# underdoc-wang/ST-MGCN

Hardware: NVIDIA H100
Metric: region-timesteps/sec (fwd+bwd) (higher is better)
Workload: dtype f32

## Files before the change

### st-mgcn_b200/csrc/lstm16.cu

```cuda
#include "tc16.cuh"
#include <cuda.h>
#include <stdlib.h>
#include <string.h>

using namespace stmgcn;
using namespace stmgcn::tc;

namespace {

constexpr int kTileM = 128;
constexpr int kHid = 64;
constexpr int kGateCols = 256;
constexpr int kMaxC = 4;
constexpr int kWTileBytes = kGateCols * 128;
constexpr int kATileBytes = kTile16Bytes;

__host__ __device__ __forceinline__ uint32_t blocked_off(uint32_t tile, uint32_t row, uint32_t unit) {
    return tile * 8192u + (unit >> 2) * 512u + row * 4u + (unit & 3u);
}
__host__ __device__ __forceinline__ int64_t blocked_slice(int n_tiles) { return (int64_t)n_tiles * kTileM * kHid; }

__device__ __forceinline__ float gate_scale(int col) { return (col & 3) == 2 ? kNeg2Log2e : kNegLog2e; }
__device__ __forceinline__ float exp_arg_(float a) { return ex2_ftz_(fminf(a, 43.28f)); }
__device__ __forceinline__ void lstm_cell_fwd8(float ai, float af, float ag, float ao, float cp, float& c, float& h) {
// ... 230 lines not shown
                    wg_wait<0>();
                }
                wg_fence_regs(acc);
            } else {
#pragma unroll
                for (int k = 0; k < 128; ++k) acc[k] = 0.f;
            }
            if (issuer) bulk_wait_group_read0();
            bar_sync(kFBarWg + wg, 128);
            if (!L0) {
                if (issuer) mbar_arrive(&tail->empty[wg]);
                ++n_below;
            }
            float* c_row = p.cs + (int64_t)t * cslice + cbase + blocked_off(0, 0, q >> 1);
            const bool store_h = valid && t == p.t_len - 1 && p.h_f32 != nullptr;
            float* h_row = p.h_f32 + (store_h ? r * (uint32_t)kHid + (uint32_t)(q >> 1) : 0u);
#pragma unroll
            for (int j0 = 0; j0 < 32; j0 += kFCellBatch) {
                float4 v[kFCellBatch], bv[kFCellBatch];
                float cp[kFCellBatch], cn[kFCellBatch], hn[kFCellBatch];
#pragma unroll
                for (int k = 0; k < kFCellBatch; ++k) v[k] = frag_to_gates(acc, j0 + k, odd);
#pragma unroll
                for (int k = 0; k < kFCellBatch; ++k) {
                    const int col = 4 * (2 * (j0 + k) + (q >> 1));
                    bv[k] = *reinterpret_cast<const float4*>(&tail->bias[col]);
                    cp[k] = c_sm[128 * (j0 + k)];
                }
#pragma unroll
                for (int k = 0; k < kFCellBatch; ++k) {
                    const int col = 4 * (2 * (j0 + k) + (q >> 1));
                    const float4 a = gate_args<CIN>(v[k], bv[k], xs, wih_s, col, kC);
                    lstm_cell_fwd8(a.x, a.y, a.z, a.w, cp[k], cn[k], hn[k]);
                }
#pragma unroll
                for (int k = 0; k < kFCellBatch; ++k) {
                    const int unit = 2 * (j0 + k) + (q >> 1);
                    c_sm[128 * (j0 + k)] = cn[k];
                    if (valid) c_row[blocked_off(0, 0, 2 * (j0 + k))] = cn[k];
                    if (store_h) h_row[2 * (j0 + k)] = hn[k];
                    const uint32_t off = sw128<2>(row_in_wg, (uint32_t)unit);
                    const __nv_bfloat16 hb = __float2bfloat16_rn(hn[k]);
                    *reinterpret_cast<__nv_bfloat16*>(h_sm + off) = hb;
                    if (PLANES == 2) *reinterpret_cast<__nv_bfloat16*>(h_sm + kHTileBytes + off) = __float2bfloat16_rn(hn[k] - __bfloat162float(hb));
                }
            }
            fence_proxy_async_smem();
            bar_sync(kFBarWg + wg, 128);
            if (issuer) {
                for (int pl = 0; pl < PLANES; ++pl)
                    tma_store_3d(&p.hp_map, h_sm + (size_t)pl * kHTileBytes, 0, row0, (p.layer * p.t_len + t) * PLANES + pl);
                bulk_commit_group();
            }
        }
    }
    if (issuer) bulk_wait_group_read0();
}

__global__ void lstm16_pack_kernel(const float* __restrict__ w_ih, const float* __restrict__ w_hh,
                                   const float* __restrict__ b_ih, const float* __restrict__ b_hh, int layer, int c_in,
                                   uint8_t* __restrict__ wimg, float* __restrict__ bias, float* __restrict__ wih_t) {
    const int nseg = layer == 0 ? 1 : 2;
    const int total = nseg * kGateCols * kHid;
    for (int e = blockIdx.x * blockDim.x + threadIdx.x; e < total; e += gridDim.x * blockDim.x) {
        const int s = e / (kGateCols * kHid), n = (e / kHid) % kGateCols, k = e % kHid;
        const int nat = (n & 3) * kHid + (n >> 2);
        const float* src = (layer > 0 && s == 0) ? w_ih : w_hh;
        const float v = src[(int64_t)nat * kHid + k];
        const __nv_bfloat16 h = __float2bfloat16_rn(v);
        const __nv_bfloat16 l = __float2bfloat16_rn(v - __bfloat162float(h));
        const uint32_t off = sw128<2>((uint32_t)n, (uint32_t)k);
        *reinterpret_cast<__nv_bfloat16*>(wimg + (size_t)(s * 2) * kWTileBytes + off) = h;
        *reinterpret_cast<__nv_bfloat16*>(wimg + (size_t)(s * 2 + 1) * kWTileBytes + off) = l;
    }
    for (int n = blockIdx.x * blockDim.x + threadIdx.x; n < kGateCols; n += gridDim.x * blockDim.x) {
        const int nat = (n & 3) * kHid + (n >> 2);
        bias[n] = b_ih[nat] + b_hh[nat];
        if (layer == 0 && wih_t != nullptr)
            for (int c = 0; c < c_in; ++c) wih_t[c * kGateCols + n] = w_ih[(int64_t)nat * c_in + c];
    }
}


constexpr int kBWarpgroups = 2;
constexpr int kBThreads = kBWarpgroups * 128 + 128;
constexpr int kBCons = kBWarpgroups * 128;
constexpr uint32_t kBBarCons = 1;
constexpr uint32_t kBBarWg = 2;
constexpr int kBDbWarps = 2;
constexpr uint32_t kBBarDa = 4;
constexpr uint32_t kBDaThreads = kBCons + 32 * kBDbWarps;
constexpr uint32_t kBConsRegs = 240, kBProdRegs = 24;
constexpr int kBATiles = 4;

struct B16Tail {
    float bias[kGateCols];
    uint64_t a_full, a_empty, w_full;
};
constexpr size_t kBSmem = 1024 + 4 * (size_t)kWTileBytes + kBATiles * (size_t)kATileBytes + 2 * (size_t)kATileBytes + sizeof(B16Tail);
static_assert(kBSmem <= 232448, "lstm16 backward kernel exceeds the 227 KB shared-memory limit");

constexpr int kBMaxSteps = 64;
struct Bwd16Step {
    int32_t slice[2];
    int8_t src[2];
    int8_t first;
    int8_t store_dh;
    int32_t t;
    const float* c_prev;
    const float* dh_in;
    float* dx_out;
};
struct Bwd16Params {
    alignas(64) CUtensorMap maps[2];
    const uint8_t* zero_tile;
    const uint8_t* wimg;
    const float* bias;
    const float* wih;
    const float* xo;
    const float* sg;
    float* d_s;
    float* d_xo;
    int c_in, t_len, n_steps;
    int64_t b_inner;
    float* dh_rec;
    float* dc;
    float* dbp;
    float* dw_slice;
    int64_t rows;
    int n_tiles;
    Bwd16Step steps[kBMaxSteps];
};
static_assert(sizeof(Bwd16Params) <= 4096, "kernel parameter block exceeds 4 KB");

template <int PLANES, int NSEG>
__device__ __forceinline__ void bwd_recompute_mma(float (&g)[32], uint32_t a_u, uint32_t a_rows, uint32_t w_u, int c) {
#pragma unroll
    for (int s = 0; s < NSEG; ++s) {
        const uint64_t a_hi = desc16_k(a_u + (uint32_t)(s * 2) * kATileBytes + a_rows);
        const uint64_t a_lo = desc16_k(a_u + (uint32_t)(s * 2 + 1) * kATileBytes + a_rows);
        const uint64_t b_hi = desc16_k(w_u + (uint32_t)(s * 2) * kWTileBytes + (uint32_t)c * 8192u);
        const uint64_t b_lo = desc16_k(w_u + (uint32_t)(s * 2 + 1) * kWTileBytes + (uint32_t)c * 8192u);
#pragma unroll
        for (int kk = 0; kk < 4; ++kk) {
            wgmma_bf16_n64_t00(g, a_hi + 2 * kk, b_hi + 2 * kk, (s > 0 || kk > 0) ? 1u : 0u);
            if (PLANES == 2) {
                wgmma_bf16_n64_t00(g, a_hi + 2 * kk, b_lo + 2 * kk, 1u);
                wgmma_bf16_n64_t00(g, a_lo + 2 * kk, b_hi + 2 * kk, 1u);
            }
        }
    }
}

constexpr uint32_t kStepMN = 2048;

template <int PLANES, bool L0>
__device__ __forceinline__ void bwd_wgrad_mma(float (&wgr)[32], uint32_t wa_hi, uint32_t da_u) {
    const uint32_t wa_lo = wa_hi + kATileBytes;
#pragma unroll
    for (int ks = 0; ks < 8; ++ks) {
        const uint64_t ah = desc16_mn(wa_hi + ks * kStepMN, kATileBytes);
        const uint64_t al = desc16_mn(wa_lo + ks * kStepMN, kATileBytes);
        const uint64_t bh = desc16_mn(da_u + ks * kStepMN, kATileBytes);
        const uint64_t bl = desc16_mn(da_u + kATileBytes + ks * kStepMN, kATileBytes);
        wgmma_bf16_n64_t11(wgr, ah, bh, ks > 0 ? 1u : 0u);
        wgmma_bf16_n64_t11(wgr, ah, bl, 1u);
        if (PLANES == 2 || L0) wgmma_bf16_n64_t11(wgr, al, bh, 1u);
    }
}

template <int PLANES, int NSEG>
__device__ __forceinline__ void bwd_dgrad_mma(float (&dacc)[32 * NSEG], uint32_t da_u, uint32_t a_rows, uint32_t w_u, int c) {
    const uint64_t ah = desc16_k(da_u + a_rows), al = desc16_k(da_u + kATileBytes + a_rows);
#pragma unroll
    for (int kk = 0; kk < 4; ++kk) {
        const uint32_t wb = w_u + (uint32_t)c * 8192u + (uint32_t)kk * kStepMN;
        const uint64_t bh = desc16_mn(wb, 2 * kWTileBytes), bl = desc16_mn(wb + kWTileBytes, 2 * kWTileBytes);
        if constexpr (NSEG == 2) {
            wgmma_bf16_n128_t01(dacc, ah + 2 * kk, bh, 1u);
            if (PLANES == 2) wgmma_bf16_n128_t01(dacc, ah + 2 * kk, bl, 1u);
            wgmma_bf16_n128_t01(dacc, al + 2 * kk, bh, 1u);
        } else {
            wgmma_bf16_n64_t01(dacc, ah + 2 * kk, bh, 1u);
            if (PLANES == 2) wgmma_bf16_n64_t01(dacc, ah + 2 * kk, bl, 1u);
            wgmma_bf16_n64_t01(dacc, al + 2 * kk, bh, 1u);
        }
    }
}

__device__ __forceinline__ void bwd_wgrad_red(float* slice, const float (&wgr)[32], uint32_t rw0, int q, int c) {
#pragma unroll
    for (int j = 0; j < 8; ++j) {
        const uint32_t n = (uint32_t)(64 * c + 8 * j + 2 * q);
        red_add_f32x2(slice + (size_t)rw0 * kGateCols + n, wgr[4 * j], wgr[4 * j + 1]);
        red_add_f32x2(slice + (size_t)(rw0 + 8) * kGateCols + n, wgr[4 * j + 2], wgr[4 * j + 3]);
    }
}

template <int PLANES, int CIN>
__global__ void __launch_bounds__(kBThreads, 1) lstm16_bwd_kernel(const __grid_constant__ Bwd16Params p) {
    constexpr bool L0 = CIN > 0;
    constexpr int kC = (CIN == 1) ? 1 : kMaxC;
    constexpr int kNseg = L0 ? 1 : 2;
    extern __shared__ uint8_t smem_raw[];
    uint8_t* smem = smem_raw + smem_pad1024(smem_raw);
    uint8_t* w_sm = smem;
    uint8_t* a_sm = w_sm + 4 * (size_t)kWTileBytes;
    uint8_t* da_sm = a_sm + kBATiles * (size_t)kATileBytes;
    B16Tail* tail = (B16Tail*)(da_sm + 2 * (size_t)kATileBytes);
    float* wih_s = reinterpret_cast<float*>(w_sm + 2 * (size_t)kWTileBytes);
    const int tid = threadIdx.x;
    const int warp = tid >> 5;
    const int lane = tid & 31;
    constexpr int kProdWarp = kBWarpgroups * 4;

    if (tid == 0) {
        mbar_init(&tail->a_full, 1);
        mbar_init(&tail->a_empty, kBWarpgroups);
        mbar_init(&tail->w_full, 1);
        fence_barrier_init();
    }
    for (int i = tid; i < kGateCols; i += kBThreads) tail->bias[i] = p.bias[i] * gate_scale(i);
    if (L0) {
        for (int i = tid; i < p.c_in * kGateCols; i += kBThreads) wih_s[i] = p.wih[i] * gate_scale(i);
        for (int i = tid; i < 2 * kATileBytes / 16; i += kBThreads)
            reinterpret_cast<uint4*>(a_sm + 2 * (size_t)kATileBytes)[i] = make_uint4(0u, 0u, 0u, 0u);
        if (PLANES == 1)
            for (int i = tid; i < kATileBytes / 16; i += kBThreads)
                reinterpret_cast<uint4*>(a_sm + (size_t)kATileBytes)[i] = make_uint4(0u, 0u, 0u, 0u);
    }
    fence_proxy_async_smem();
    __syncthreads();
    const int my_tiles = cta_tiles(p.n_tiles);
    const int n_items = my_tiles * p.n_steps;

    if (warp >= kProdWarp) {
        setmaxnreg_dec<kBProdRegs>();
        const bool leader = warp == kProdWarp && elect_one_sync();
        if (leader && n_items > 0) {
            load_weights<kNseg, PLANES>(w_sm, p, &tail->w_full);
            const uint64_t once = l2_evict_first();
            for (int w = 0; w < n_items; ++w) {
                const int ti = w / p.n_steps, st = w - ti * p.n_steps, tile = cta_tile(ti);
                const Bwd16Step& sp = p.steps[st];
                mbar_wait_polite(&tail->a_empty, (uint32_t)(w & 1) ^ 1u);
                mbar_arrive_expect_tx(&tail->a_full, (uint32_t)(kNseg * PLANES * kATileBytes));
                for (int sg = 0; sg < kNseg; ++sg)
                    for (int pl = 0; pl < PLANES; ++pl) {
                        uint8_t* dst = a_sm + (size_t)(sg * 2 + pl) * kATileBytes;
                        if (sp.src[sg] == 2) bulk_g2s(dst, p.zero_tile, kATileBytes, &tail->a_full);
                        else tma_load_3d_hint(dst, &p.maps[sp.src[sg]], 0, tile * kTileM, sp.slice[sg] + pl, &tail->a_full, once);
                    }
                const int64_t o = (int64_t)tile * kTileM * kHid;
                constexpr uint32_t kB = kTileM * kHid * 4;
                if (sp.c_prev) prefetch_l2(sp.c_prev + o, kB);
                if (sp.dh_in) prefetch_l2(sp.dh_in + o, kB);
                if (w + 1 < n_items) {
                    const int ti1 = (w + 1) / p.n_steps, tile1 = cta_tile(ti1);
                    const Bwd16Step& sp1 = p.steps[w + 1 - ti1 * p.n_steps];
                    for (int sg = 0; sg < kNseg; ++sg)
                        for (int pl = 0; pl < PLANES; ++pl)
                            if (sp1.src[sg] != 2) tma_prefetch_3d(&p.maps[sp1.src[sg]], 0, tile1 * kTileM, sp1.slice[sg] + pl);
                }
            }
        } else if (warp > kProdWarp && warp <= kProdWarp + kBDbWarps && n_items > 0) {
            const uint8_t* rows = da_sm + (size_t)(warp - kProdWarp - 1) * 64u * 128u;
            float db[4][2] = {};
            for (int w = 0; w < n_items; ++w) {
#pragma unroll
                for (int c = 0; c < 4; ++c) {
                    bar_sync(kBBarDa, kBDaThreads);
                    bar_sync(kBBarDa, kBDaThreads);
#pragma unroll 1
                    for (uint32_t r4 = 0; r4 < 64u; r4 += 4u) {
#pragma unroll
                        for (uint32_t k = 0; k < 4; ++k) {
                            const uint32_t off = sw128<2>(r4 + k, 2u * (uint32_t)lane);
                            const uint32_t hi = *reinterpret_cast<const uint32_t*>(rows + off);
                            const uint32_t lo = *reinterpret_cast<const uint32_t*>(rows + kATileBytes + off);
                            db[c][0] += bf16_lo_as_f32(hi) + bf16_lo_as_f32(lo);
                            db[c][1] += bf16_hi_as_f32(hi) + bf16_hi_as_f32(lo);
                        }
                    }
                }
            }
#pragma unroll
            for (int c = 0; c < 4; ++c) {
                atomicAdd(&p.dbp[64 * c + 2 * lane], db[c][0]);
                atomicAdd(&p.dbp[64 * c + 2 * lane + 1], db[c][1]);
            }
        }
        return;
    }

    setmaxnreg_inc<kBConsRegs>();
    const int wg = tid >> 7;
    const int q = lane & 3;
    const bool odd = (q & 1) != 0;
    const uint32_t rw0 = (uint32_t)(64 * wg + 16 * (warp & 3) + (lane >> 2));
    const uint32_t row_in_tile = rw0 + (odd ? 8u : 0u);
    const uint32_t rows32 = (uint32_t)p.rows;
    const uint32_t w_u = smem_u32(w_sm), a_u = smem_u32(a_sm), da_u = smem_u32(da_sm);
    const uint32_t a_rows = (uint32_t)wg * 64u * 128u;
    const uint32_t wa_u = a_u + (uint32_t)(wg * 2) * kATileBytes;
    float* slice = p.dw_slice + (size_t)blockIdx.x * (kTileM * kGateCols);
    mbar_wait_raw(&tail->w_full, 0);

    for (int w = 0; w < n_items; ++w) {
        const int ti = w / p.n_steps, st = w - ti * p.n_steps, tile = cta_tile(ti);
        const Bwd16Step& sp = p.steps[st];
        const uint32_t r = (uint32_t)tile * kTileM + row_in_tile;
        const bool valid = r < rows32;
        float xs[kMaxC], xraw[kMaxC], dxs[kMaxC];
        if (L0) {
            const float sv = valid ? p.sg[(r % (uint32_t)p.b_inner) * (uint32_t)p.t_len + (uint32_t)sp.t] : 0.f;
#pragma unroll
            for (int c = 0; c < kMaxC; ++c) {
                xraw[c] = (c < kC && valid && (CIN == 1 || c < p.c_in)) ? p.xo[((int64_t)r * p.t_len + sp.t) * p.c_in + c] : 0.f;
                xs[c] = xraw[c] * sv;
                dxs[c] = 0.f;
            }
        }
        bar_sync(kBBarCons, kBCons);
        if (L0 && (q >> 1) == 0) {
            uint32_t hi[2], lo[2];
            split_bf16x2(xs[0], xs[1], hi[0], lo[0]);
            split_bf16x2(xs[2], xs[3], hi[1], lo[1]);
            const uint32_t off = sw128<2>(row_in_tile, 0);
            *reinterpret_cast<uint2*>(a_sm + 2 * (size_t)kATileBytes + off) = make_uint2(hi[0], hi[1]);
            *reinterpret_cast<uint2*>(a_sm + 3 * (size_t)kATileBytes + off) = make_uint2(lo[0], lo[1]);
        }
        mbar_wait_raw(&tail->a_full, (uint32_t)w & 1u);
        float dacc[32 * kNseg];
#pragma unroll
        for (int k = 0; k < 32 * kNseg; ++k) dacc[k] = 0.f;
        float wgr[32];
        const uint32_t bo = blocked_off(tile, row_in_tile, 0);
        float cpv[8], dhv[8], dciv[8];
        auto load_cells = [&](int c) {
            float dhr[8];
#pragma unroll
            for (int j = 0; j < 8; ++j) {
                const int unit = 16 * c + 2 * j + (q >> 1);
                const uint32_t o = bo + blocked_off(0, 0, unit);
                const bool rec = valid && !sp.first;
                cpv[j] = (valid && sp.c_prev) ? __ldcs(sp.c_prev + o) : 0.f;
                dhv[j] = (valid && sp.dh_in) ? __ldcs(sp.dh_in + o) : 0.f;
                dhr[j] = rec ? p.dh_rec[o] : 0.f;
                dciv[j] = rec ? p.dc[o] : 0.f;
            }
#pragma unroll
            for (int j = 0; j < 8; ++j) dhv[j] += dhr[j];
        };
        uint32_t dpk[32];
        auto cell_epilogue = [&](int c, const float (&g)[32]) {
#pragma unroll
            for (int j = 0; j < 8; ++j) {
                const float4 v = frag_to_gates(g, j, odd);
                const int unit = 16 * c + 2 * j + (q >> 1);
                const int col = 4 * unit;
                const float4 bv = *reinterpret_cast<const float4*>(&tail->bias[col]);
                const float4 a = gate_args<CIN>(v, bv, xs, wih_s, col, p.c_in);
                const uint32_t o = bo + blocked_off(0, 0, unit);
                const float cp = cpv[j], dh = dhv[j], dci = dciv[j];
                float gi, gf, gg, go, tc_;
                lstm_cell_gates8(a.x, a.y, a.z, a.w, cp, gi, gf, gg, go, tc_);
                const float dcv = fmaf(dh * go, 1.f - tc_ * tc_, dci);
                const float da0 = dcv * gg * gi * (1.f - gi);
                const float da1 = dcv * cp * gf * (1.f - gf);
                const float da2 = dcv * gi * (1.f - gg * gg);
                const float da3 = dh * tc_ * go * (1.f - go);
                if (valid) p.dc[o] = dcv * gf;
                if (L0) {
#pragma unroll
                    for (int cc = 0; cc < kC; ++cc)
                        if (CIN == 1 || cc < p.c_in) {
                            const float4 wv = *reinterpret_cast<const float4*>(&wih_s[cc * kGateCols + col]);
                            dxs[cc] = fmaf(da0 * wv.x + da1 * wv.y + 0.5f * (da2 * wv.z) + da3 * wv.w, -kLn2, dxs[cc]);
                        }
                }
                split_bf16x2(da0, da1, dpk[4 * j], dpk[4 * j + 2]);
                split_bf16x2(da2, da3, dpk[4 * j + 1], dpk[4 * j + 3]);
            }
        };
        auto store_da = [&]() {
            bar_sync(kBBarDa, kBDaThreads);
#pragma unroll
            for (int j = 0; j < 8; ++j) {
                const uint32_t off = sw128<2>(row_in_tile, 4 * (2 * j + (q >> 1)));
                *reinterpret_cast<uint2*>(da_sm + off) = make_uint2(dpk[4 * j], dpk[4 * j + 1]);
                *reinterpret_cast<uint2*>(da_sm + kATileBytes + off) = make_uint2(dpk[4 * j + 2], dpk[4 * j + 3]);
            }
            fence_proxy_async_smem();
            bar_sync(kBBarDa, kBDaThreads);
        };
        {
            float g[32];
            wg_fence_regs(g);
            wg_fence();
            bwd_recompute_mma<PLANES, kNseg>(g, a_u, a_rows, w_u, 0);
            wg_commit();
            load_cells(0);
            wg_wait<0>();
            wg_fence_regs(g);
            cell_epilogue(0, g);
            store_da();
        }
#pragma unroll 1
        for (int c = 1; c < 4; ++c) {
            uint32_t a_c = a_u, w_c = w_u, wa_c = wa_u, da_c = da_u;
            asm volatile("" : "+r"(a_c), "+r"(w_c), "+r"(wa_c), "+r"(da_c));
            float g[32];
            wg_fence_regs(g);
            wg_fence_regs(wgr);
            wg_fence_regs(dacc);
            wg_fence();
            bwd_recompute_mma<PLANES, kNseg>(g, a_c, a_rows, w_c, c);
            wg_commit();
            bwd_wgrad_mma<PLANES, L0>(wgr, wa_c, da_c);
            bwd_dgrad_mma<PLANES, kNseg>(dacc, da_c, a_rows, w_c, c - 1);
            wg_commit();
            load_cells(c);
            wg_wait<1>();
            wg_fence_regs(g);
            cell_epilogue(c, g);
            wg_wait<0>();
            wg_fence_regs(wgr);
            wg_fence_regs(dacc);
            bwd_wgrad_red(slice, wgr, rw0, q, c - 1);
            store_da();
        }
        wg_fence_regs(wgr);
        wg_fence_regs(dacc);
        wg_fence();
        bwd_wgrad_mma<PLANES, L0>(wgr, wa_u, da_u);
        wg_commit();
        bwd_dgrad_mma<PLANES, kNseg>(dacc, da_u, a_rows, w_u, 3);
        wg_commit();
        wg_wait<1>();
        wg_fence_regs(wgr);
        bar_sync(kBBarWg + wg, 128);
        if ((tid & 127) == 0) mbar_arrive(&tail->a_empty);
        bwd_wgrad_red(slice, wgr, rw0, q, 3);
        wg_wait<0>();
        wg_fence_regs(dacc);
#pragma unroll
        for (int h = 0; h < 2; ++h) {
            const uint32_t rr = rw0 + 8u * h;
            if ((uint32_t)tile * kTileM + rr >= rows32) continue;
#pragma unroll
            for (int j = 0; j < 8 * kNseg; ++j) {
                const int col = 8 * j + 2 * q;
                const bool is_dx = !L0 && col < 64;
                float* base = is_dx ? sp.dx_out : p.dh_rec;
                if (base == nullptr || !(is_dx || sp.store_dh)) continue;
                const int unit = col & 63;
                *reinterpret_cast<float2*>(base + (uint32_t)tile * 8192u + (uint32_t)(unit >> 2) * 512u + rr * 4u + (uint32_t)(unit & 3)) =
                    make_float2(dacc[4 * j + 2 * h], dacc[4 * j + 2 * h + 1]);
            }
        }
        if (L0) {
            float contrib = 0.f;
#pragma unroll
            for (int cc = 0; cc < kC; ++cc) contrib += dxs[cc] * xraw[cc];
            contrib += __shfl_xor_sync(0xffffffffu, contrib, 2);
            if ((q >> 1) == 0 && valid) atomicAdd(&p.d_s[(int64_t)(r % (uint32_t)p.b_inner) * p.t_len + sp.t], contrib);
            if (p.d_xo != nullptr) {
                float* dst = p.d_xo + ((int64_t)r * p.t_len + sp.t) * p.c_in;
                const float sv = valid ? p.sg[(r % (uint32_t)p.b_inner) * (uint32_t)p.t_len + (uint32_t)sp.t] : 0.f;
#pragma unroll
                for (int cc = 0; cc < kC; ++cc) {
                    const float dx = dxs[cc] + __shfl_xor_sync(0xffffffffu, dxs[cc], 2);
                    if ((q >> 1) == 0 && valid && (CIN == 1 || cc < p.c_in)) dst[cc] = dx * sv;
                }
            }
        }
    }
}

__global__ void lstm16_wgrad_reduce_kernel(const float* __restrict__ slices, int n_slices, int layer, int c_in,
                                           const float* __restrict__ dbp, float* __restrict__ d_w_ih,
                                           float* __restrict__ d_w_hh, float* __restrict__ d_b_ih, float* __restrict__ d_b_hh) {
    const int e = blockIdx.x * blockDim.x + threadIdx.x;
    if (e < kTileM * kGateCols) {
        float s = 0.f;
        for (int i = 0; i < n_slices; ++i) s += slices[(size_t)i * (kTileM * kGateCols) + e];
        const int m = e / kGateCols, n = e % kGateCols;
        const int nat = (n & 3) * kHid + (n >> 2);
        if (layer > 0) {
            if (m < 64) d_w_ih[(size_t)nat * kHid + m] = s;
            else d_w_hh[(size_t)nat * kHid + (m - 64)] = s;
        } else {
            if (m < 64) d_w_hh[(size_t)nat * kHid + m] = s;
            else if (m - 64 < c_in) d_w_ih[(size_t)nat * c_in + (m - 64)] = s;
        }
    }
    if (e < kGateCols) {
        const int nat = (e & 3) * kHid + (e >> 2);
        d_b_ih[nat] = dbp[e];
        d_b_hh[nat] = dbp[e];
    }
}

}

namespace stmgcn {

typedef CUresult (*EncodeTiledFn16)(CUtensorMap*, CUtensorMapDataType, cuuint32_t, void*, const cuuint64_t*, const cuuint64_t*,
                                    const cuuint32_t*, const cuuint32_t*, CUtensorMapInterleave, CUtensorMapSwizzle,
                                    CUtensorMapL2promotion, CUtensorMapFloatOOBfill);
static EncodeTiledFn16 encode_fn16() {
    static EncodeTiledFn16 fn = nullptr;
    static bool tried = false;
    if (!tried) {
        tried = true;
        void* sym = nullptr;
        cudaDriverEntryPointQueryResult qres;
        if (cudaGetDriverEntryPoint("cuTensorMapEncodeTiled", &sym, cudaEnableDefault, &qres) == cudaSuccess &&
            qres == cudaDriverEntryPointSuccess)
            fn = (EncodeTiledFn16)sym;
    }
    return fn;
}
static bool make_plane_map(CUtensorMap* map, const void* base, int64_t rows, int64_t slices, int box_rows) {
    EncodeTiledFn16 fn = encode_fn16();
    if (fn == nullptr) return false;
    const cuuint64_t dims[3] = {(cuuint64_t)kHid, (cuuint64_t)rows, (cuuint64_t)slices};
    const cuuint64_t strides[2] = {(cuuint64_t)kHid * 2, (cuuint64_t)rows * kHid * 2};
    const cuuint32_t box[3] = {(cuuint32_t)kHid, (cuuint32_t)box_rows, 1};
    const cuuint32_t estr[3] = {1, 1, 1};
    return fn(map, CU_TENSOR_MAP_DATA_TYPE_BFLOAT16, 3, const_cast<void*>(base), dims, strides, box, estr,
              CU_TENSOR_MAP_INTERLEAVE_NONE, CU_TENSOR_MAP_SWIZZLE_128B, CU_TENSOR_MAP_L2_PROMOTION_NONE,
              CU_TENSOR_MAP_FLOAT_OOB_FILL_NONE) == CUDA_SUCCESS;
}
static int32_t make_plane_maps(const char* who, CUtensorMap* hp_map, CUtensorMap* h0_map, const void* hp, const void* h0p,
                               int64_t rows, int n_layers, int t_len, int planes, int box_rows) {
    STMGCN_REQUIRE(make_plane_map(hp_map, hp, rows, (int64_t)n_layers * t_len * planes, box_rows), STMGCN_ERR_STATE,
                   "%s: cuTensorMapEncodeTiled failed (hp)", who);
    if (h0p != nullptr)
        STMGCN_REQUIRE(make_plane_map(h0_map, h0p, rows, (int64_t)n_layers * planes, box_rows), STMGCN_ERR_STATE,
                       "%s: cuTensorMapEncodeTiled failed (h0p)", who);
    return 0;
}

static int32_t check_dims16(const char* who, int32_t t_len, int32_t n_layers, int64_t rows, int32_t c_in, int64_t b_inner,
                            int32_t planes, const float* wih_t, const void* h0p, const float* c0) {
    STMGCN_REQUIRE(planes == 1 || planes == 2, STMGCN_ERR_ARG, "%s: planes=%d", who, planes);
    STMGCN_REQUIRE(n_layers >= 1 && n_layers <= 8 && t_len >= 1 && rows > 0 && c_in >= 1 && c_in <= kMaxC && b_inner > 0,
                   STMGCN_ERR_SHAPE, "%s: L=%d T=%d rows=%lld C=%d", who, n_layers, t_len, (long long)rows, c_in);
    STMGCN_REQUIRE(rows <= (1LL << 25), STMGCN_ERR_SHAPE, "%s: rows=%lld too large (32-bit element offsets)", who, (long long)rows);
    STMGCN_REQUIRE((h0p == nullptr) == (c0 == nullptr), STMGCN_ERR_ARG, "%s: h0p and c0 go together", who);
    STMGCN_REQUIRE(wih_t != nullptr, STMGCN_ERR_ARG, "%s: wih_t null", who);
    return 0;
}

static int64_t wimg_off(int l) { return (int64_t)2 * kWTileBytes * (l == 0 ? 0 : 2 * l - 1); }

template <int N> struct Int { static constexpr int value = N; };
// ... 164 lines not shown
```

Before: 46.69 million.

## Overlap next step's first recompute MMA with current step's dgrad store in LSTM backward

Restructures the backward LSTM consumer loop so the first chunk's gate-recompute MMA for the next work item is issued before the current item's dgrad accumulator is written out. Cell loads are split into the item's own inputs and the recurrent dh part, and the recurrent part waits on a consumer-wide barrier after the dh stores. This hides the epilogue store latency and the per-item prologue behind tensor-core work. In exchange it uses a full-consumer barrier where per-warpgroup barriers were used before, adds more live state across iterations, and re-reads x for the L0 reduction.

```diff
diff --git a/st-mgcn_b200/csrc/lstm16.cu b/st-mgcn_b200/csrc/lstm16.cu
--- a/st-mgcn_b200/csrc/lstm16.cu
+++ b/st-mgcn_b200/csrc/lstm16.cu
@@ -340,7 +340,6 @@
 constexpr int kBThreads = kBWarpgroups * 128 + 128;
 constexpr int kBCons = kBWarpgroups * 128;
 constexpr uint32_t kBBarCons = 1;
-constexpr uint32_t kBBarWg = 2;
 constexpr int kBDbWarps = 2;
 constexpr uint32_t kBBarDa = 4;
 constexpr uint32_t kBDaThreads = kBCons + 32 * kBDbWarps;
@@ -560,104 +559,147 @@
     float* slice = p.dw_slice + (size_t)blockIdx.x * (kTileM * kGateCols);
     mbar_wait_raw(&tail->w_full, 0);
 
+    struct Row { int tile; const Bwd16Step* sp; uint32_t r, bo; bool valid; };
+    auto row_of = [&](int w) {
+        const int ti = w / p.n_steps;
+        Row x;
+        x.tile = cta_tile(ti);
+        x.sp = &p.steps[w - ti * p.n_steps];
+        x.r = (uint32_t)x.tile * kTileM + row_in_tile;
+        x.valid = x.r < rows32;
+        x.bo = blocked_off(x.tile, row_in_tile, 0);
+        return x;
+    };
+    float xs[kMaxC], dxs[kMaxC];
+    auto load_x = [&](const Row& x, float (&xr)[kMaxC]) {
+#pragma unroll
+        for (int c = 0; c < kMaxC; ++c)
+            xr[c] = (c < kC && x.valid && (CIN == 1 || c < p.c_in)) ? p.xo[((int64_t)x.r * p.t_len + x.sp->t) * p.c_in + c] : 0.f;
+    };
+    auto s_of = [&](const Row& x) {
+        return x.valid ? p.sg[(x.r % (uint32_t)p.b_inner) * (uint32_t)p.t_len + (uint32_t)x.sp->t] : 0.f;
+    };
+    auto enter = [&](const Row& x) {
+        if (L0) {
+            float xr[kMaxC];
+            load_x(x, xr);
+            const float sv = s_of(x);
+#pragma unroll
+            for (int c = 0; c < kMaxC; ++c) {
+                xs[c] = xr[c] * sv;
+                dxs[c] = 0.f;
+            }
+            if ((q >> 1) == 0) {
+                uint32_t hi[2], lo[2];
+                split_bf16x2(xs[0], xs[1], hi[0], lo[0]);
+                split_bf16x2(xs[2], xs[3], hi[1], lo[1]);
+                const uint32_t off = sw128<2>(row_in_tile, 0);
+                *reinterpret_cast<uint2*>(a_sm + 2 * (size_t)kATileBytes + off) = make_uint2(hi[0], hi[1]);
+                *reinterpret_cast<uint2*>(a_sm + 3 * (size_t)kATileBytes + off) = make_uint2(lo[0], lo[1]);
+            }
+        }
+    };
+    float dacc[32 * kNseg];
+#pragma unroll
+    for (int k = 0; k < 32 * kNseg; ++k) dacc[k] = 0.f;
+    float wgr[32];
+    float cpv[8], dhv[8], dciv[8];
+    constexpr int kCellsAll = 0, kCellsOwn = 1, kCellsRec = 2;
+    auto load_cells = [&](const Row& x, int c, int part) {
+        float dhr[8];
+#pragma unroll
+        for (int j = 0; j < 8; ++j) {
+            const int unit = 16 * c + 2 * j + (q >> 1);
+            const uint32_t o = x.bo + blocked_off(0, 0, unit);
+            const bool rec = x.valid && !x.sp->first;
+            if (part != kCellsRec) {
+                cpv[j] = (x.valid && x.sp->c_prev) ? __ldcs(x.sp->c_prev + o) : 0.f;
+                dhv[j] = (x.valid && x.sp->dh_in) ? __ldcs(x.sp->dh_in + o) : 0.f;
+                dciv[j] = rec ? p.dc[o] : 0.f;
+            }
+            if (part != kCellsOwn) dhr[j] = rec ? p.dh_rec[o] : 0.f;
+        }
+        if (part != kCellsOwn)
+#pragma unroll
+            for (int j = 0; j < 8; ++j) dhv[j] += dhr[j];
+    };
+    uint32_t dpk[32];
+    auto cell_epilogue = [&](const Row& x, int c, const float (&g)[32]) {
+#pragma unroll
+        for (int j = 0; j < 8; ++j) {
+            const float4 v = frag_to_gates(g, j, odd);
+            const int unit = 16 * c + 2 * j + (q >> 1);
+            const int col = 4 * unit;
+            const float4 bv = *reinterpret_cast<const float4*>(&tail->bias[col]);
+            const float4 a = gate_args<CIN>(v, bv, xs, wih_s, col, p.c_in);
+            const uint32_t o = x.bo + blocked_off(0, 0, unit);
+            const float cp = cpv[j], dh = dhv[j], dci = dciv[j];
+            float gi, gf, gg, go, tc_;
+            lstm_cell_gates8(a.x, a.y, a.z, a.w, cp, gi, gf, gg, go, tc_);
+            const float dcv = fmaf(dh * go, 1.f - tc_ * tc_, dci);
+            const float da0 = dcv * gg * gi * (1.f - gi);
+            const float da1 = dcv * cp * gf * (1.f - gf);
+            const float da2 = dcv * gi * (1.f - gg * gg);
+            const float da3 = dh * tc_ * go * (1.f - go);
+            if (x.valid) p.dc[o] = dcv * gf;
+            if (L0) {
+#pragma unroll
+                for (int cc = 0; cc < kC; ++cc)
+                    if (CIN == 1 || cc < p.c_in) {
+                        const float4 wv = *reinterpret_cast<const float4*>(&wih_s[cc * kGateCols + col]);
+                        dxs[cc] = fmaf(da0 * wv.x + da1 * wv.y + 0.5f * (da2 * wv.z) + da3 * wv.w, -kLn2, dxs[cc]);
+                    }
+            }
+            split_bf16x2(da0, da1, dpk[4 * j], dpk[4 * j + 2]);
+            split_bf16x2(da2, da3, dpk[4 * j + 1], dpk[4 * j + 3]);
+        }
+    };
+    auto store_da = [&]() {
+        bar_sync(kBBarDa, kBDaThreads);
+#pragma unroll
+        for (int j = 0; j < 8; ++j) {
+            const uint32_t off = sw128<2>(row_in_tile, 4 * (2 * j + (q >> 1)));
+            *reinterpret_cast<uint2*>(da_sm + off) = make_uint2(dpk[4 * j], dpk[4 * j + 1]);
+            *reinterpret_cast<uint2*>(da_sm + kATileBytes + off) = make_uint2(dpk[4 * j + 2], dpk[4 * j + 3]);
+        }
+        fence_proxy_async_smem();
+        bar_sync(kBBarDa, kBDaThreads);
+    };
+    auto store_dacc = [&](const Row& x) {
+#pragma unroll
+        for (int h = 0; h < 2; ++h) {
+            const uint32_t rr = rw0 + 8u * h;
+            if ((uint32_t)x.tile * kTileM + rr >= rows32) continue;
+#pragma unroll
+            for (int j = 0; j < 8 * kNseg; ++j) {
+                const int col = 8 * j + 2 * q;
+                const bool is_dx = !L0 && col < 64;
+                float* base = is_dx ? x.sp->dx_out : p.dh_rec;
+                if (base == nullptr || !(is_dx || x.sp->store_dh)) continue;
+                const int unit = col & 63;
+                *reinterpret_cast<float2*>(base + (uint32_t)x.tile * 8192u + (uint32_t)(unit >> 2) * 512u + rr * 4u + (uint32_t)(unit & 3)) =
+                    make_float2(dacc[4 * j + 2 * h], dacc[4 * j + 2 * h + 1]);
+            }
+        }
+#pragma unroll
+        for (int k = 0; k < 32 * kNseg; ++k) dacc[k] = 0.f;
+    };
+
+
+    if (n_items > 0) enter(row_of(0));
     for (int w = 0; w < n_items; ++w) {
-        const int ti = w / p.n_steps, st = w - ti * p.n_steps, tile = cta_tile(ti);
-        const Bwd16Step& sp = p.steps[st];
-        const uint32_t r = (uint32_t)tile * kTileM + row_in_tile;
-        const bool valid = r < rows32;
-        float xs[kMaxC], xraw[kMaxC], dxs[kMaxC];
-        if (L0) {
-            const float sv = valid ? p.sg[(r % (uint32_t)p.b_inner) * (uint32_t)p.t_len + (uint32_t)sp.t] : 0.f;
-#pragma unroll
-            for (int c = 0; c < kMaxC; ++c) {
-                xraw[c] = (c < kC && valid && (CIN == 1 || c < p.c_in)) ? p.xo[((int64_t)r * p.t_len + sp.t) * p.c_in + c] : 0.f;
-                xs[c] = xraw[c] * sv;
-                dxs[c] = 0.f;
-            }
-        }
-        bar_sync(kBBarCons, kBCons);
-        if (L0 && (q >> 1) == 0) {
-            uint32_t hi[2], lo[2];
-            split_bf16x2(xs[0], xs[1], hi[0], lo[0]);
-            split_bf16x2(xs[2], xs[3], hi[1], lo[1]);
-            const uint32_t off = sw128<2>(row_in_tile, 0);
-            *reinterpret_cast<uint2*>(a_sm + 2 * (size_t)kATileBytes + off) = make_uint2(hi[0], hi[1]);
-            *reinterpret_cast<uint2*>(a_sm + 3 * (size_t)kATileBytes + off) = make_uint2(lo[0], lo[1]);
-        }
-        mbar_wait_raw(&tail->a_full, (uint32_t)w & 1u);
-        float dacc[32 * kNseg];
-#pragma unroll
-        for (int k = 0; k < 32 * kNseg; ++k) dacc[k] = 0.f;
-        float wgr[32];
-        const uint32_t bo = blocked_off(tile, row_in_tile, 0);
-        float cpv[8], dhv[8], dciv[8];
-        auto load_cells = [&](int c) {
-            float dhr[8];
-#pragma unroll
-            for (int j = 0; j < 8; ++j) {
-                const int unit = 16 * c + 2 * j + (q >> 1);
-                const uint32_t o = bo + blocked_off(0, 0, unit);
-                const bool rec = valid && !sp.first;
-                cpv[j] = (valid && sp.c_prev) ? __ldcs(sp.c_prev + o) : 0.f;
-                dhv[j] = (valid && sp.dh_in) ? __ldcs(sp.dh_in + o) : 0.f;
-                dhr[j] = rec ? p.dh_rec[o] : 0.f;
-                dciv[j] = rec ? p.dc[o] : 0.f;
-            }
-#pragma unroll
-            for (int j = 0; j < 8; ++j) dhv[j] += dhr[j];
-        };
-        uint32_t dpk[32];
-        auto cell_epilogue = [&](int c, const float (&g)[32]) {
-#pragma unroll
-            for (int j = 0; j < 8; ++j) {
-                const float4 v = frag_to_gates(g, j, odd);
-                const int unit = 16 * c + 2 * j + (q >> 1);
-                const int col = 4 * unit;
-                const float4 bv = *reinterpret_cast<const float4*>(&tail->bias[col]);
-                const float4 a = gate_args<CIN>(v, bv, xs, wih_s, col, p.c_in);
-                const uint32_t o = bo + blocked_off(0, 0, unit);
-                const float cp = cpv[j], dh = dhv[j], dci = dciv[j];
-                float gi, gf, gg, go, tc_;
-                lstm_cell_gates8(a.x, a.y, a.z, a.w, cp, gi, gf, gg, go, tc_);
-                const float dcv = fmaf(dh * go, 1.f - tc_ * tc_, dci);
-                const float da0 = dcv * gg * gi * (1.f - gi);
-                const float da1 = dcv * cp * gf * (1.f - gf);
-                const float da2 = dcv * gi * (1.f - gg * gg);
-                const float da3 = dh * tc_ * go * (1.f - go);
-                if (valid) p.dc[o] = dcv * gf;
-                if (L0) {
-#pragma unroll
-                    for (int cc = 0; cc < kC; ++cc)
-                        if (CIN == 1 || cc < p.c_in) {
-                            const float4 wv = *reinterpret_cast<const float4*>(&wih_s[cc * kGateCols + col]);
-                            dxs[cc] = fmaf(da0 * wv.x + da1 * wv.y + 0.5f * (da2 * wv.z) + da3 * wv.w, -kLn2, dxs[cc]);
-                        }
-                }
-                split_bf16x2(da0, da1, dpk[4 * j], dpk[4 * j + 2]);
-                split_bf16x2(da2, da3, dpk[4 * j + 1], dpk[4 * j + 3]);
-            }
-        };
-        auto store_da = [&]() {
-            bar_sync(kBBarDa, kBDaThreads);
-#pragma unroll
-            for (int j = 0; j < 8; ++j) {
-                const uint32_t off = sw128<2>(row_in_tile, 4 * (2 * j + (q >> 1)));
-                *reinterpret_cast<uint2*>(da_sm + off) = make_uint2(dpk[4 * j], dpk[4 * j + 1]);
-                *reinterpret_cast<uint2*>(da_sm + kATileBytes + off) = make_uint2(dpk[4 * j + 2], dpk[4 * j + 3]);
-            }
-            fence_proxy_async_smem();
-            bar_sync(kBBarDa, kBDaThreads);
-        };
-        {
+        const Row x = row_of(w);
+        if (w == 0) {
+            mbar_wait_raw(&tail->a_full, 0u);
             float g[32];
             wg_fence_regs(g);
             wg_fence();
             bwd_recompute_mma<PLANES, kNseg>(g, a_u, a_rows, w_u, 0);
             wg_commit();
-            load_cells(0);
+            load_cells(x, 0, kCellsAll);
             wg_wait<0>();
             wg_fence_regs(g);
-            cell_epilogue(0, g);
+            cell_epilogue(x, 0, g);
             store_da();
         }
 #pragma unroll 1
@@ -674,10 +716,10 @@
             bwd_wgrad_mma<PLANES, L0>(wgr, wa_c, da_c);
             bwd_dgrad_mma<PLANES, kNseg>(dacc, da_c, a_rows, w_c, c - 1);
             wg_commit();
-            load_cells(c);
+            load_cells(x, c, kCellsAll);
             wg_wait<1>();
             wg_fence_regs(g);
-            cell_epilogue(c, g);
+            cell_epilogue(x, c, g);
             wg_wait<0>();
             wg_fence_regs(wgr);
             wg_fence_regs(dacc);
@@ -693,41 +735,52 @@
         wg_commit();
         wg_wait<1>();
         wg_fence_regs(wgr);
-        bar_sync(kBBarWg + wg, 128);
+        bar_sync(kBBarCons, kBCons);
         if ((tid & 127) == 0) mbar_arrive(&tail->a_empty);
         bwd_wgrad_red(slice, wgr, rw0, q, 3);
-        wg_wait<0>();
-        wg_fence_regs(dacc);
-#pragma unroll
-        for (int h = 0; h < 2; ++h) {
-            const uint32_t rr = rw0 + 8u * h;
-            if ((uint32_t)tile * kTileM + rr >= rows32) continue;
-#pragma unroll
-            for (int j = 0; j < 8 * kNseg; ++j) {
-                const int col = 8 * j + 2 * q;
-                const bool is_dx = !L0 && col < 64;
-                float* base = is_dx ? sp.dx_out : p.dh_rec;
-                if (base == nullptr || !(is_dx || sp.store_dh)) continue;
-                const int unit = col & 63;
-                *reinterpret_cast<float2*>(base + (uint32_t)tile * 8192u + (uint32_t)(unit >> 2) * 512u + rr * 4u + (uint32_t)(unit & 3)) =
-                    make_float2(dacc[4 * j + 2 * h], dacc[4 * j + 2 * h + 1]);
-            }
-        }
         if (L0) {
+            float xr[kMaxC];
+            load_x(x, xr);
             float contrib = 0.f;
 #pragma unroll
-            for (int cc = 0; cc < kC; ++cc) contrib += dxs[cc] * xraw[cc];
+            for (int cc = 0; cc < kC; ++cc) contrib += dxs[cc] * xr[cc];
             contrib += __shfl_xor_sync(0xffffffffu, contrib, 2);
-            if ((q >> 1) == 0 && valid) atomicAdd(&p.d_s[(int64_t)(r % (uint32_t)p.b_inner) * p.t_len + sp.t], contrib);
+            if ((q >> 1) == 0 && x.valid) atomicAdd(&p.d_s[(int64_t)(x.r % (uint32_t)p.b_inner) * p.t_len + x.sp->t], contrib);
             if (p.d_xo != nullptr) {
-                float* dst = p.d_xo + ((int64_t)r * p.t_len + sp.t) * p.c_in;
-                const float sv = valid ? p.sg[(r % (uint32_t)p.b_inner) * (uint32_t)p.t_len + (uint32_t)sp.t] : 0.f;
+                float* dst = p.d_xo + ((int64_t)x.r * p.t_len + x.sp->t) * p.c_in;
+                const float sv = s_of(x);
 #pragma unroll
                 for (int cc = 0; cc < kC; ++cc) {
                     const float dx = dxs[cc] + __shfl_xor_sync(0xffffffffu, dxs[cc], 2);
-                    if ((q >> 1) == 0 && valid && (CIN == 1 || cc < p.c_in)) dst[cc] = dx * sv;
+                    if ((q >> 1) == 0 && x.valid && (CIN == 1 || cc < p.c_in)) dst[cc] = dx * sv;
                 }
             }
+        }
+        if (w + 1 < n_items) {
+            const Row x1 = row_of(w + 1);
+            enter(x1);
+            mbar_wait_raw(&tail->a_full, (uint32_t)(w + 1) & 1u);
+            uint32_t a_c = a_u, w_c = w_u;
+            asm volatile("" : "+r"(a_c), "+r"(w_c));
+            float g[32];
+            wg_fence_regs(g);
+            wg_fence();
+            bwd_recompute_mma<PLANES, kNseg>(g, a_c, a_rows, w_c, 0);
+            wg_commit();
+            load_cells(x1, 0, kCellsOwn);
+            wg_wait<1>();
+            wg_fence_regs(dacc);
+            store_dacc(x);
+            bar_sync(kBBarCons, kBCons);
+            load_cells(x1, 0, kCellsRec);
+            wg_wait<0>();
+            wg_fence_regs(g);
+            cell_epilogue(x1, 0, g);
+            store_da();
+        } else {
+            wg_wait<0>();
+            wg_fence_regs(dacc);
+            store_dacc(x);
         }
     }
 }
```

Measured after the change: 47.29 million (median of 6 runs). 1.3% higher.

## Specialize LSTM backward warps into cell and gradient warpgroups with mbarrier pipeline

Applied to the files above, without the earlier changes.

Splits the backward kernel's consumer warpgroups into two cell warpgroups, which recompute gates and produce dA, and a dedicated gradient warpgroup that runs the weight-grad and data-grad WGMMAs and stores dh/dx. Named barriers between consumers are replaced by mbarriers (da_full, da_empty, dh_ready), so cell math for chunk c can overlap gradient MMAs for the previous chunk. Register budgets are rebalanced per role. The gradient warpgroup now writes dh_rec, so the cell warps must wait on dh_ready before reading it. That adds cross-role latency on the recurrent dependency and single-buffered dA handoff stalls.

```diff
diff --git a/st-mgcn_b200/csrc/lstm16.cu b/st-mgcn_b200/csrc/lstm16.cu
--- a/st-mgcn_b200/csrc/lstm16.cu
+++ b/st-mgcn_b200/csrc/lstm16.cu
@@ -336,20 +336,18 @@
 }
 
 
-constexpr int kBWarpgroups = 2;
-constexpr int kBThreads = kBWarpgroups * 128 + 128;
-constexpr int kBCons = kBWarpgroups * 128;
-constexpr uint32_t kBBarCons = 1;
-constexpr uint32_t kBBarWg = 2;
+constexpr int kBCellWgs = 2;
+constexpr int kBGradWarp = kBCellWgs * 4;
+constexpr int kBProdWarp = kBGradWarp + 4;
+constexpr int kBThreads = kBProdWarp * 32 + 128;
 constexpr int kBDbWarps = 2;
-constexpr uint32_t kBBarDa = 4;
-constexpr uint32_t kBDaThreads = kBCons + 32 * kBDbWarps;
-constexpr uint32_t kBConsRegs = 240, kBProdRegs = 24;
+constexpr uint32_t kBCellRegs = 136, kBGradRegs = 200, kBProdRegs = 40;
 constexpr int kBATiles = 4;
 
 struct B16Tail {
     float bias[kGateCols];
     uint64_t a_full, a_empty, w_full;
+    uint64_t da_full, da_empty, dh_ready;
 };
 constexpr size_t kBSmem = 1024 + 4 * (size_t)kWTileBytes + kBATiles * (size_t)kATileBytes + 2 * (size_t)kATileBytes + sizeof(B16Tail);
 static_assert(kBSmem <= 232448, "lstm16 backward kernel exceeds the 227 KB shared-memory limit");
@@ -442,12 +440,11 @@
     }
 }
 
-__device__ __forceinline__ void bwd_wgrad_red(float* slice, const float (&wgr)[32], uint32_t rw0, int q, int c) {
+__device__ __forceinline__ void bwd_wgrad_red(float* frag, const float (&wgr)[32], int c) {
 #pragma unroll
     for (int j = 0; j < 8; ++j) {
-        const uint32_t n = (uint32_t)(64 * c + 8 * j + 2 * q);
-        red_add_f32x2(slice + (size_t)rw0 * kGateCols + n, wgr[4 * j], wgr[4 * j + 1]);
-        red_add_f32x2(slice + (size_t)(rw0 + 8) * kGateCols + n, wgr[4 * j + 2], wgr[4 * j + 3]);
+        red_add_f32x2(frag + 64 * c + 8 * j, wgr[4 * j], wgr[4 * j + 1]);
+        red_add_f32x2(frag + 8 * kGateCols + 64 * c + 8 * j, wgr[4 * j + 2], wgr[4 * j + 3]);
     }
 }
 
@@ -466,12 +463,14 @@
     const int tid = threadIdx.x;
     const int warp = tid >> 5;
     const int lane = tid & 31;
-    constexpr int kProdWarp = kBWarpgroups * 4;
 
     if (tid == 0) {
         mbar_init(&tail->a_full, 1);
-        mbar_init(&tail->a_empty, kBWarpgroups);
+        mbar_init(&tail->a_empty, 4 * (kBCellWgs + 1));
         mbar_init(&tail->w_full, 1);
+        mbar_init(&tail->da_full, 4 * kBCellWgs);
+        mbar_init(&tail->da_empty, 4 + kBDbWarps);
+        mbar_init(&tail->dh_ready, 128);
         fence_barrier_init();
     }
     for (int i = tid; i < kGateCols; i += kBThreads) tail->bias[i] = p.bias[i] * gate_scale(i);
@@ -487,10 +486,12 @@
     __syncthreads();
     const int my_tiles = cta_tiles(p.n_tiles);
     const int n_items = my_tiles * p.n_steps;
-
-    if (warp >= kProdWarp) {
+    const uint32_t rows32 = (uint32_t)p.rows;
+    const uint32_t w_u = smem_u32(w_sm), a_u = smem_u32(a_sm), da_u = smem_u32(da_sm);
+
+    if (warp >= kBProdWarp) {
         setmaxnreg_dec<kBProdRegs>();
-        const bool leader = warp == kProdWarp && elect_one_sync();
+        const bool leader = warp == kBProdWarp && elect_one_sync();
         if (leader && n_items > 0) {
             load_weights<kNseg, PLANES>(w_sm, p, &tail->w_full);
             const uint64_t once = l2_evict_first();
@@ -517,14 +518,13 @@
                             if (sp1.src[sg] != 2) tma_prefetch_3d(&p.maps[sp1.src[sg]], 0, tile1 * kTileM, sp1.slice[sg] + pl);
                 }
             }
-        } else if (warp > kProdWarp && warp <= kProdWarp + kBDbWarps && n_items > 0) {
-            const uint8_t* rows = da_sm + (size_t)(warp - kProdWarp - 1) * 64u * 128u;
+        } else if (warp > kBProdWarp && warp <= kBProdWarp + kBDbWarps && n_items > 0) {
+            const uint8_t* rows = da_sm + (size_t)(warp - kBProdWarp - 1) * 64u * 128u;
             float db[4][2] = {};
             for (int w = 0; w < n_items; ++w) {
 #pragma unroll
                 for (int c = 0; c < 4; ++c) {
-                    bar_sync(kBBarDa, kBDaThreads);
-                    bar_sync(kBBarDa, kBDaThreads);
+                    mbar_wait_raw(&tail->da_full, (uint32_t)c & 1u);
 #pragma unroll 1
                     for (uint32_t r4 = 0; r4 < 64u; r4 += 4u) {
 #pragma unroll
@@ -536,6 +536,8 @@
                             db[c][1] += bf16_hi_as_f32(hi) + bf16_hi_as_f32(lo);
                         }
                     }
+                    __syncwarp();
+                    if (elect_one_sync()) mbar_arrive(&tail->da_empty);
                 }
             }
 #pragma unroll
@@ -547,18 +549,79 @@
         return;
     }
 
-    setmaxnreg_inc<kBConsRegs>();
+    const int q = lane & 3;
+    mbar_wait_raw(&tail->w_full, 0);
+
+    if (warp >= kBGradWarp) {
+        setmaxnreg_inc<kBGradRegs>();
+        const uint32_t fr = (uint32_t)(16 * (warp & 3) + (lane >> 2));
+        float* frag = p.dw_slice + (size_t)blockIdx.x * (kTileM * kGateCols) + fr * kGateCols + 2 * q;
+        for (int w = 0; w < n_items; ++w) {
+            const int ti = w / p.n_steps, st = w - ti * p.n_steps, tile = cta_tile(ti);
+            const Bwd16Step& sp = p.steps[st];
+            float dacc[2][32 * kNseg];
+#pragma unroll
+            for (int k = 0; k < 32 * kNseg; ++k) dacc[0][k] = dacc[1][k] = 0.f;
+            mbar_wait_raw(&tail->a_full, (uint32_t)w & 1u);
+#pragma unroll 1
+            for (int c = 0; c < 4; ++c) {
+                uint32_t a_c = a_u, w_c = w_u, da_c = da_u;
+                asm volatile("" : "+r"(a_c), "+r"(w_c), "+r"(da_c));
+                float wgr[32];
+                mbar_wait_raw(&tail->da_full, (uint32_t)c & 1u);
+                wg_fence_regs(wgr);
+                wg_fence();
+                bwd_wgrad_mma<PLANES, L0>(wgr, a_c, da_c);
+                wg_commit();
+                wg_wait<0>();
+                wg_fence_regs(wgr);
+                bwd_wgrad_red(frag, wgr, c);
+                wg_fence_regs(wgr);
+                wg_fence_regs(dacc[0]);
+                wg_fence_regs(dacc[1]);
+                wg_fence();
+                bwd_wgrad_mma<PLANES, L0>(wgr, a_c + 2u * kATileBytes, da_c);
+                wg_commit();
+                bwd_dgrad_mma<PLANES, kNseg>(dacc[0], da_c, 0u, w_c, c);
+                bwd_dgrad_mma<PLANES, kNseg>(dacc[1], da_c, 64u * 128u, w_c, c);
+                wg_commit();
+                wg_wait<1>();
+                wg_fence_regs(wgr);
+                if (c == 3 && elect_one_sync()) mbar_arrive(&tail->a_empty);
+                bwd_wgrad_red(frag + 64 * kGateCols, wgr, c);
+                wg_wait<0>();
+                wg_fence_regs(dacc[0]);
+                wg_fence_regs(dacc[1]);
+                if (elect_one_sync()) mbar_arrive(&tail->da_empty);
+            }
+            auto store_cols = [&](float* base, int j0, int j1) {
+#pragma unroll
+                for (int half = 0; half < 2; ++half) {
+#pragma unroll
+                    for (int h = 0; h < 2; ++h) {
+                        const uint32_t rr = 64u * half + fr + 8u * h;
+                        if ((uint32_t)tile * kTileM + rr >= rows32) continue;
+#pragma unroll
+                        for (int j = j0; j < j1; ++j) {
+                            const int unit = (8 * j + 2 * q) & 63;
+                            *reinterpret_cast<float2*>(base + (uint32_t)tile * 8192u + (uint32_t)(unit >> 2) * 512u + rr * 4u + (uint32_t)(unit & 3)) =
+                                make_float2(dacc[half][4 * j + 2 * h], dacc[half][4 * j + 2 * h + 1]);
+                        }
+                    }
+                }
+            };
+            if (sp.store_dh) store_cols(p.dh_rec, 8 * (kNseg - 1), 8 * kNseg);
+            mbar_arrive(&tail->dh_ready);
+            if (!L0 && sp.dx_out != nullptr) store_cols(sp.dx_out, 0, 8);
+        }
+        return;
+    }
+
+    setmaxnreg_inc<kBCellRegs>();
     const int wg = tid >> 7;
-    const int q = lane & 3;
     const bool odd = (q & 1) != 0;
-    const uint32_t rw0 = (uint32_t)(64 * wg + 16 * (warp & 3) + (lane >> 2));
-    const uint32_t row_in_tile = rw0 + (odd ? 8u : 0u);
-    const uint32_t rows32 = (uint32_t)p.rows;
-    const uint32_t w_u = smem_u32(w_sm), a_u = smem_u32(a_sm), da_u = smem_u32(da_sm);
+    const uint32_t row_in_tile = (uint32_t)(64 * wg + 16 * (warp & 3) + (lane >> 2)) + (odd ? 8u : 0u);
     const uint32_t a_rows = (uint32_t)wg * 64u * 128u;
-    const uint32_t wa_u = a_u + (uint32_t)(wg * 2) * kATileBytes;
-    float* slice = p.dw_slice + (size_t)blockIdx.x * (kTileM * kGateCols);
-    mbar_wait_raw(&tail->w_full, 0);
 
     for (int w = 0; w < n_items; ++w) {
         const int ti = w / p.n_steps, st = w - ti * p.n_steps, tile = cta_tile(ti);
@@ -575,7 +638,7 @@
                 dxs[c] = 0.f;
             }
         }
-        bar_sync(kBBarCons, kBCons);
+        mbar_wait_raw(&tail->a_full, (uint32_t)w & 1u);
         if (L0 && (q >> 1) == 0) {
             uint32_t hi[2], lo[2];
             split_bf16x2(xs[0], xs[1], hi[0], lo[0]);
@@ -584,25 +647,21 @@
             *reinterpret_cast<uint2*>(a_sm + 2 * (size_t)kATileBytes + off) = make_uint2(hi[0], hi[1]);
             *reinterpret_cast<uint2*>(a_sm + 3 * (size_t)kATileBytes + off) = make_uint2(lo[0], lo[1]);
         }
-        mbar_wait_raw(&tail->a_full, (uint32_t)w & 1u);
-        float dacc[32 * kNseg];
-#pragma unroll
-        for (int k = 0; k < 32 * kNseg; ++k) dacc[k] = 0.f;
-        float wgr[32];
         const uint32_t bo = blocked_off(tile, row_in_tile, 0);
         float cpv[8], dhv[8], dciv[8];
+        const bool rec = valid && !sp.first;
         auto load_cells = [&](int c) {
             float dhr[8];
 #pragma unroll
             for (int j = 0; j < 8; ++j) {
-                const int unit = 16 * c + 2 * j + (q >> 1);
-                const uint32_t o = bo + blocked_off(0, 0, unit);
-                const bool rec = valid && !sp.first;
+                const uint32_t o = bo + blocked_off(0, 0, 16 * c + 2 * j + (q >> 1));
                 cpv[j] = (valid && sp.c_prev) ? __ldcs(sp.c_prev + o) : 0.f;
                 dhv[j] = (valid && sp.dh_in) ? __ldcs(sp.dh_in + o) : 0.f;
-                dhr[j] = rec ? p.dh_rec[o] : 0.f;
                 dciv[j] = rec ? p.dc[o] : 0.f;
             }
+            if (c == 0 && st > 0) mbar_wait_raw(&tail->dh_ready, (uint32_t)(w - 1) & 1u);
+#pragma unroll
+            for (int j = 0; j < 8; ++j) dhr[j] = rec ? p.dh_rec[bo + blocked_off(0, 0, 16 * c + 2 * j + (q >> 1))] : 0.f;
 #pragma unroll
             for (int j = 0; j < 8; ++j) dhv[j] += dhr[j];
         };
@@ -637,8 +696,21 @@
                 split_bf16x2(da2, da3, dpk[4 * j + 1], dpk[4 * j + 3]);
             }
         };
-        auto store_da = [&]() {
-            bar_sync(kBBarDa, kBDaThreads);
+#pragma unroll 1
+        for (int c = 0; c < 4; ++c) {
+            uint32_t a_c = a_u, w_c = w_u;
+            asm volatile("" : "+r"(a_c), "+r"(w_c));
+            float g[32];
+            wg_fence_regs(g);
+            wg_fence();
+            bwd_recompute_mma<PLANES, kNseg>(g, a_c, a_rows, w_c, c);
+            wg_commit();
+            load_cells(c);
+            wg_wait<0>();
+            wg_fence_regs(g);
+            if (c == 3 && elect_one_sync()) mbar_arrive(&tail->a_empty);
+            cell_epilogue(c, g);
+            mbar_wait_raw(&tail->da_empty, (uint32_t)(c & 1) ^ 1u);
 #pragma unroll
             for (int j = 0; j < 8; ++j) {
                 const uint32_t off = sw128<2>(row_in_tile, 4 * (2 * j + (q >> 1)));
@@ -646,72 +718,8 @@
                 *reinterpret_cast<uint2*>(da_sm + kATileBytes + off) = make_uint2(dpk[4 * j + 2], dpk[4 * j + 3]);
             }
             fence_proxy_async_smem();
-            bar_sync(kBBarDa, kBDaThreads);
-        };
-        {
-            float g[32];
-            wg_fence_regs(g);
-            wg_fence();
-            bwd_recompute_mma<PLANES, kNseg>(g, a_u, a_rows, w_u, 0);
-            wg_commit();
-            load_cells(0);
-            wg_wait<0>();
-            wg_fence_regs(g);
-            cell_epilogue(0, g);
-            store_da();
-        }
-#pragma unroll 1
-        for (int c = 1; c < 4; ++c) {
-            uint32_t a_c = a_u, w_c = w_u, wa_c = wa_u, da_c = da_u;
-            asm volatile("" : "+r"(a_c), "+r"(w_c), "+r"(wa_c), "+r"(da_c));
-            float g[32];
-            wg_fence_regs(g);
-            wg_fence_regs(wgr);
-            wg_fence_regs(dacc);
-            wg_fence();
-            bwd_recompute_mma<PLANES, kNseg>(g, a_c, a_rows, w_c, c);
-            wg_commit();
-            bwd_wgrad_mma<PLANES, L0>(wgr, wa_c, da_c);
-            bwd_dgrad_mma<PLANES, kNseg>(dacc, da_c, a_rows, w_c, c - 1);
-            wg_commit();
-            load_cells(c);
-            wg_wait<1>();
-            wg_fence_regs(g);
-            cell_epilogue(c, g);
-            wg_wait<0>();
-            wg_fence_regs(wgr);
-            wg_fence_regs(dacc);
-            bwd_wgrad_red(slice, wgr, rw0, q, c - 1);
-            store_da();
-        }
-        wg_fence_regs(wgr);
-        wg_fence_regs(dacc);
-        wg_fence();
-        bwd_wgrad_mma<PLANES, L0>(wgr, wa_u, da_u);
-        wg_commit();
-        bwd_dgrad_mma<PLANES, kNseg>(dacc, da_u, a_rows, w_u, 3);
-        wg_commit();
-        wg_wait<1>();
-        wg_fence_regs(wgr);
-        bar_sync(kBBarWg + wg, 128);
-        if ((tid & 127) == 0) mbar_arrive(&tail->a_empty);
-        bwd_wgrad_red(slice, wgr, rw0, q, 3);
-        wg_wait<0>();
-        wg_fence_regs(dacc);
-#pragma unroll
-        for (int h = 0; h < 2; ++h) {
-            const uint32_t rr = rw0 + 8u * h;
-            if ((uint32_t)tile * kTileM + rr >= rows32) continue;
-#pragma unroll
-            for (int j = 0; j < 8 * kNseg; ++j) {
-                const int col = 8 * j + 2 * q;
-                const bool is_dx = !L0 && col < 64;
-                float* base = is_dx ? sp.dx_out : p.dh_rec;
-                if (base == nullptr || !(is_dx || sp.store_dh)) continue;
-                const int unit = col & 63;
-                *reinterpret_cast<float2*>(base + (uint32_t)tile * 8192u + (uint32_t)(unit >> 2) * 512u + rr * 4u + (uint32_t)(unit & 3)) =
-                    make_float2(dacc[4 * j + 2 * h], dacc[4 * j + 2 * h + 1]);
-            }
+            __syncwarp();
+            if (elect_one_sync()) mbar_arrive(&tail->da_full);
         }
         if (L0) {
             float contrib = 0.f;
```

Result: faster. 47.47 million before, 50.03 million after (median of 6 runs) (+5.4%).
